# zju3dv/pats

Measured on AMD Instinct MI355X. Metric: image-pairs/sec (coarse+fine OT) on 640x480 MegaDepth; OT iters/sec per pair, higher is better.
Workload: dtype f32 (contractions: fp32 operands split into fp16 hi + lo, three exact-product MFMA passes, fp32 accumulate)

## Files before the change

### include/pats_amd.h

```cpp
#ifndef PATS_AMD_H
#define PATS_AMD_H

#include <stddef.h>
#include <stdint.h>

#ifdef __cplusplus
extern "C" {
#endif

typedef void* pats_stream_t;

enum {
    PATS_OK = 0,
    PATS_ERR_INVALID = 1,
    PATS_ERR_UNSUPPORTED = 2,
    PATS_ERR_LAUNCH = 3,
    PATS_ERR_NO_DEVICE = 4
};

enum { PATS_SINKHORN_AUTO = 0, PATS_SINKHORN_LOG = 1, PATS_SINKHORN_KERNEL = 2 };

const char* pats_version(void);
#define PATS_ABI_VERSION 8
int pats_abi_version(void);
const char* pats_last_error(void);
int pats_device_count(void);
int pats_set_sinkhorn_mode(int mode);
int pats_set_fine_fused(int on);

int pats_set_third_gather(int mode);

int pats_sinkhorn_fallbacks(int64_t* count, int reset);

int pats_sinkhorn_tail_solves(int64_t* count, int reset);

int pats_cost_f32(const float* d0, const float* d1, int64_t batch, int D, int n, int m, float* out,
                  pats_stream_t stream);

size_t pats_sinkhorn_workspace_bytes(int64_t batch, int M, int N);
int pats_sinkhorn_f32(const float* Z, int64_t batch, int M, int N, const float* log_mu,
                      const float* log_nu, int iters, float* out, void* workspace,
                      size_t workspace_bytes, pats_stream_t stream);

size_t pats_ot_workspace_bytes(int64_t batch, int M, int N);
int pats_log_optimal_transport_f32(const float* scores, int64_t batch, int m, int n,
                                   const float* alpha, const float* ns, int iters, float* Z,
                                   void* workspace, size_t workspace_bytes, pats_stream_t stream);

size_t pats_ot2_workspace_bytes(int64_t batch, int m, int n);
int pats_log_optimal_transport2_flags_f32(const float* scores, int64_t batch, int m, int n,
                                          const float* one, const float* ns, int iters, float bias_k,
                                          float* Z, uint8_t* col_nomatch, void* workspace,
                                          size_t workspace_bytes, pats_stream_t stream);
int pats_log_optimal_transport2_f32(const float* scores, int64_t batch, int m, int n,
                                    const float* one, const float* ns, int iters, float bias_k,
                                    float* Z, void* workspace, size_t workspace_bytes,
                                    pats_stream_t stream);

int pats_cost_ot_f32(const float* d0, const float* d1, int64_t batch, int D, int n, int m,
                     int variant, const float* scalar, const float* ns, int iters, float bias_k,
                     float* Z, void* workspace, size_t workspace_bytes, pats_stream_t stream);
size_t pats_cost_ot_workspace_bytes(int64_t batch, int D, int n, int m, int variant);
int pats_cost_ot_flags_f32(const float* d0, const float* d1, int64_t batch, int D, int n, int m,
                           int variant, const float* scalar, const float* ns, int iters, float bias_k,
                           float* Z, uint8_t* col_nomatch, void* workspace, size_t workspace_bytes,
                           pats_stream_t stream);

int pats_set_cost_ot_mid_event(void* event);

int pats_cost_ot_flags_counted_f32(const float* d0, const float* d1, int64_t batch_cap, const int64_t* batch_dev,
                                   int D, int n, int m, int variant, const float* scalar, const float* ns, int iters,
                                   float bias_k, float* Z, uint8_t* col_nomatch, void* workspace,
                                   size_t workspace_bytes, pats_stream_t stream);

int pats_colmass_sqrt_f32(const float* Z, int64_t batch, int M, int N, float* out,
                          pats_stream_t stream);
int pats_colmass_flags_f32(const float* Z, int64_t batch, int M, int N, float* out, uint8_t* col_nomatch,
                           pats_stream_t stream);
int pats_dustbin_bias_inplace_f32(float* Z, int64_t batch, int M, int N, float k,
                                  pats_stream_t stream);
int pats_exp_f32(const float* Z, int64_t count, float* out, pats_stream_t stream);

int pats_argmax_f32(const float* Z, int64_t batch, int M, int N, int64_t* row_arg,
                    int64_t* col_arg, pats_stream_t stream);

int pats_iterative_expand_f32(const float* P, int input_is_log, int64_t batch, int M, int N,
                              const float* scalex, const float* scaley, int lim3, int h, int w,
                              float lower_bound, int iter_num, float* whole_cost, float* core_cost,
                              float* average_point, float* x_scale, float* y_scale, int64_t* bound,
                              uint8_t* row_nomatch, pats_stream_t stream);

int pats_iterative_expand_counted_f32(const float* P, int input_is_log, int64_t batch_cap, const int64_t* batch_dev,
                                      int M, int N, const float* scalex, const float* scaley, int lim3, int h, int w,
                                      float lower_bound, int iter_num, float* whole_cost, float* core_cost,
                                      float* average_point, float* x_scale, float* y_scale, int64_t* bound,
                                      uint8_t* row_nomatch, pats_stream_t stream);

int pats_split_patches(const int32_t* sum_cycle_host, int height, int width, int max_once_used,
                       int64_t* second_layer_set, int64_t* third_layer_set);
int pats_split_patches_device(const int32_t* sum_cycle, int64_t pairs, int height, int width,
                              int max_once_used, int64_t* second_layer_set, int64_t* third_layer_set,
                              int32_t* cycle_num, pats_stream_t stream);

int pats_compute_imgs_bounds_f32(const float* x_scale, const float* y_scale,
                                 const float* average_point, const uint8_t* if_nomatching, int Np,
                                 int height, int width, int img, int64_t* bound5, int64_t* K_out,
                                 float* x_scale_new, float* y_scale_new, float* average_new,
                                 pats_stream_t stream);

int pats_left_crops_f32(const float* left, int n_img, int H, int W, const int64_t* bound5, int64_t K,
                        int height, int width, float* out, pats_stream_t stream);

int pats_compute_imgs_bounds_batch_f32(const float* x_scale, const float* y_scale, const float* average_point,
// ... 471 lines not shown
```

### pats_amd/_lib.py

```python
import ctypes
import os

_HERE = os.path.dirname(os.path.abspath(__file__))
LIB_PATH = os.path.join(_HERE, "libpats_amd.so")
if os.environ.get("PATS_AMD_DIAG_LIB", "") not in ("", "0"):
    _sfx = os.environ["PATS_AMD_DIAG_LIB"]
    LIB_PATH = os.path.join(_HERE, "libpats_amd_diag%s.so" % ("" if _sfx == "1" else _sfx))

c_void_p, c_int, c_i64, c_f, c_size = (ctypes.c_void_p, ctypes.c_int, ctypes.c_int64, ctypes.c_float,
                                       ctypes.c_size_t)

ABI_VERSION = 8



class PairTable(ctypes.Structure):
    _fields_ = [("pairs", ctypes.c_int64), ("shape_host", c_void_p), ("cell_base_host", c_void_p), ("shape", c_void_p),
                ("cell_base", c_void_p), ("img_base", c_void_p)]


_TAB = ctypes.POINTER(PairTable)


class CropFormat(ctypes.Structure):
    _fields_ = [("dtype", ctypes.c_int32), ("layout", ctypes.c_int32), ("normalize", ctypes.c_int32),
                ("mean", ctypes.c_float * 3), ("std", ctypes.c_float * 3)]


_FMT = ctypes.POINTER(CropFormat)

_SCORE_ARGS = [c_void_p, c_void_p, c_void_p, c_void_p, c_i64, c_void_p, c_i64, c_i64, c_void_p, c_i64, c_void_p, c_void_p, c_int, c_f,
               c_void_p, c_void_p, c_void_p, c_void_p, c_void_p, c_void_p, c_size, c_void_p]
_ADAPTIVE_ARGS = [ctypes.c_double, c_int, c_int, c_i64, c_void_p, c_void_p]
_POLISH_ARGS = [c_void_p, c_void_p, c_void_p, c_void_p, c_i64, c_void_p, c_i64, c_i64, c_void_p, c_void_p, c_int, c_f, c_void_p, c_i64,
                c_void_p, c_int, c_void_p, c_void_p, c_void_p, c_void_p, c_void_p, c_void_p, c_void_p, c_size, c_void_p]

SIGNATURES = {
    "pats_version": (ctypes.c_char_p, []),
    "pats_abi_version": (c_int, []),
    "pats_last_error": (ctypes.c_char_p, []),
    "pats_device_count": (c_int, []),
    "pats_set_sinkhorn_mode": (c_int, [c_int]),
    "pats_set_fine_fused": (c_int, [c_int]),
    "pats_set_third_gather": (c_int, [c_int]),
    "pats_sinkhorn_fallbacks": (c_int, [ctypes.POINTER(ctypes.c_int64), c_int]),
    "pats_sinkhorn_tail_solves": (c_int, [ctypes.POINTER(ctypes.c_int64), c_int]),
    "pats_set_gnn_redo_mode": (c_int, [c_int]),
    "pats_gnn_overflows": (c_int, [ctypes.POINTER(ctypes.c_int64), c_int]),
    "pats_cost_f32": (c_int, [c_void_p, c_void_p, c_i64, c_int, c_int, c_int, c_void_p, c_void_p]),
    "pats_sinkhorn_workspace_bytes": (c_size, [c_i64, c_int, c_int]),
    "pats_sinkhorn_f32": (c_int, [c_void_p, c_i64, c_int, c_int, c_void_p, c_void_p, c_int, c_void_p,
                                  c_void_p, c_size, c_void_p]),
    "pats_ot_workspace_bytes": (c_size, [c_i64, c_int, c_int]),
    "pats_log_optimal_transport_f32": (c_int, [c_void_p, c_i64, c_int, c_int, c_void_p, c_void_p, c_int,
                                               c_void_p, c_void_p, c_size, c_void_p]),
    "pats_ot2_workspace_bytes": (c_size, [c_i64, c_int, c_int]),
    "pats_log_optimal_transport2_f32": (c_int, [c_void_p, c_i64, c_int, c_int, c_void_p, c_void_p, c_int,
                                                c_f, c_void_p, c_void_p, c_size, c_void_p]),
    "pats_cost_ot_f32": (c_int, [c_void_p, c_void_p, c_i64, c_int, c_int, c_int, c_int, c_void_p,
                                 c_void_p, c_int, c_f, c_void_p, c_void_p, c_size, c_void_p]),
    "pats_cost_ot_flags_f32": (c_int, [c_void_p, c_void_p, c_i64, c_int, c_int, c_int, c_int, c_void_p,
                                       c_void_p, c_int, c_f, c_void_p, c_void_p, c_void_p, c_size, c_void_p]),
    "pats_set_cost_ot_mid_event": (c_int, [c_void_p]),
    "pats_cost_ot_flags_counted_f32": (c_int, [c_void_p, c_void_p, c_i64, c_void_p, c_int, c_int, c_int, c_int, c_void_p,
                                               c_void_p, c_int, c_f, c_void_p, c_void_p, c_void_p, c_size, c_void_p]),
    "pats_iterative_expand_counted_f32": (c_int, [c_void_p, c_int, c_i64, c_void_p, c_int, c_int, c_void_p, c_void_p, c_int,
                                                  c_int, c_int, c_f, c_int, c_void_p, c_void_p, c_void_p,
                                                  c_void_p, c_void_p, c_void_p, c_void_p, c_void_p]),
    "pats_fine_descriptors_counted_f32": (c_int, [c_void_p, c_void_p, c_void_p, c_void_p, c_void_p, c_i64, c_void_p, c_int,
                                                  c_void_p, c_void_p]),
    "pats_log_optimal_transport2_flags_f32": (c_int, [c_void_p, c_i64, c_int, c_int, c_void_p, c_void_p, c_int,
                                                      c_f, c_void_p, c_void_p, c_void_p, c_size, c_void_p]),
    "pats_colmass_flags_f32": (c_int, [c_void_p, c_i64, c_int, c_int, c_void_p, c_void_p, c_void_p]),
    "pats_cost_ot_workspace_bytes": (c_size, [c_i64, c_int, c_int, c_int, c_int]),
    "pats_colmass_sqrt_f32": (c_int, [c_void_p, c_i64, c_int, c_int, c_void_p, c_void_p]),
    "pats_dustbin_bias_inplace_f32": (c_int, [c_void_p, c_i64, c_int, c_int, c_f, c_void_p]),
    "pats_exp_f32": (c_int, [c_void_p, c_i64, c_void_p, c_void_p]),
    "pats_argmax_f32": (c_int, [c_void_p, c_i64, c_int, c_int, c_void_p, c_void_p, c_void_p]),
    "pats_iterative_expand_f32": (c_int, [c_void_p, c_int, c_i64, c_int, c_int, c_void_p, c_void_p, c_int,
                                          c_int, c_int, c_f, c_int, c_void_p, c_void_p, c_void_p,
                                          c_void_p, c_void_p, c_void_p, c_void_p, c_void_p]),
    "pats_split_patches": (c_int, [c_void_p, c_int, c_int, c_int, c_void_p, c_void_p]),
    "pats_split_patches_device": (c_int, [c_void_p, c_i64, c_int, c_int, c_int, c_void_p, c_void_p, c_void_p, c_void_p]),
    "pats_compute_imgs_bounds_batch_f32": (c_int, [c_void_p, c_void_p, c_void_p, c_void_p, c_int, c_int, c_int, c_int,
                                                   c_void_p, c_void_p, c_void_p, c_void_p, c_void_p, c_void_p, c_void_p]),
    "pats_left_crops_counted_f32": (c_int, [c_void_p, c_int, c_int, c_int, c_void_p, c_i64, c_void_p, c_int, c_int,
                                            c_void_p, c_void_p]),
    "pats_tensor_resize_hwc_counted_f32": (c_int, [c_void_p, c_int, c_int, c_int, c_int, c_void_p, c_i64, c_void_p,
                                                   c_void_p, c_void_p, c_void_p]),
    "pats_compute_imgs_bounds_f32": (c_int, [c_void_p, c_void_p, c_void_p, c_void_p, c_int, c_int, c_int,
                                             c_int, c_void_p, c_void_p, c_void_p, c_void_p, c_void_p,
                                             c_void_p]),
    "pats_left_crops_f32": (c_int, [c_void_p, c_int, c_int, c_int, c_void_p, c_i64, c_int, c_int, c_void_p,
                                    c_void_p]),
    "pats_tensor_resize_f32": (c_int, [c_void_p, c_int, c_int, c_int, c_int, c_void_p, c_i64, c_void_p,
                                       c_void_p, c_void_p]),
    "pats_tensor_resize_hwc_f32": (c_int, [c_void_p, c_int, c_int, c_int, c_int, c_void_p, c_i64,
                                           c_void_p, c_void_p, c_void_p]),
    "pats_compute_result_f32": (c_int, [c_void_p, c_int, c_i64, c_void_p, c_void_p, c_void_p, c_void_p,
                                        c_int, c_void_p, c_void_p, c_void_p, c_void_p, c_void_p,
                                        c_void_p]),
    "pats_compute_result_ws_f32": (c_int, [c_void_p, c_int, c_i64, c_void_p, c_void_p, c_void_p, c_void_p,
                                           c_int, c_void_p, c_void_p, c_void_p, c_void_p, c_void_p,
                                           c_void_p, c_size, c_void_p]),
    "pats_fine_descriptors_f32": (c_int, [c_void_p, c_void_p, c_void_p, c_void_p, c_void_p, c_i64, c_void_p, c_void_p]),
    "pats_third_descriptors_f32": (c_int, [c_void_p, c_void_p, c_void_p, c_void_p, c_void_p, c_void_p, c_void_p,
                                           c_i64, c_i64, c_void_p, c_void_p, c_void_p, c_void_p, c_void_p]),
    "pats_third_level_f32": (c_int, [c_void_p, c_void_p, c_i64, c_int, c_void_p, c_void_p, c_void_p, c_void_p,
                                     c_void_p, c_int, c_int, c_void_p, c_void_p, c_void_p, c_void_p, c_void_p,
                                     c_void_p]),
    "pats_third_descriptors_counted_f32": (c_int, [c_void_p, c_void_p, c_void_p, c_void_p, c_void_p, c_void_p, c_void_p,
                                                   c_i64, c_void_p, c_i64, c_void_p, c_void_p, c_void_p, c_void_p, c_void_p]),
    "pats_fine_descriptors_nhwc_f32": (c_int, [c_void_p, c_void_p, c_void_p, c_void_p, c_void_p, c_i64, c_void_p, c_void_p]),
    "pats_third_descriptors_nhwc_f32": (c_int, [c_void_p, c_void_p, c_void_p, c_void_p, c_void_p, c_void_p, c_void_p,
                                                c_i64, c_void_p, c_i64, c_void_p, c_void_p, c_void_p, c_void_p, c_void_p]),
    "pats_fine_descriptors_typed": (c_int, [c_void_p, c_void_p, c_void_p, c_int, c_int, c_void_p, c_void_p, c_i64, c_void_p,
                                            c_void_p, c_void_p]),
    "pats_third_descriptors_typed": (c_int, [c_void_p, c_void_p, c_int, c_int, c_void_p, c_void_p, c_void_p, c_void_p, c_void_p,
                                             c_i64, c_void_p, c_i64, c_void_p, c_void_p, c_void_p, c_void_p, c_void_p]),
    "pats_fine_descriptors_typed_out": (c_int, [c_void_p, c_void_p, c_void_p, c_int, c_int, c_void_p, c_void_p, c_i64, c_void_p,
                                                c_void_p, c_int, c_void_p]),
    "pats_third_descriptors_typed_out": (c_int, [c_void_p, c_void_p, c_int, c_int, c_void_p, c_void_p, c_void_p, c_void_p,
                                                 c_void_p, c_i64, c_void_p, c_i64, c_void_p, c_void_p, c_int, c_void_p, c_void_p,
                                                 c_void_p]),
    "pats_third_level_counted_f32": (c_int, [c_void_p, c_void_p, c_i64, c_void_p, c_int, c_void_p, c_void_p, c_void_p,
                                             c_void_p, c_void_p, c_int, c_int, c_void_p, c_void_p, c_void_p, c_void_p,
                                             c_void_p]),
# ... 107 lines not shown
    "pats_epipolar_pose_by_pair_f64": (c_int, [c_void_p, c_void_p, c_void_p, c_void_p, c_i64, c_void_p, c_i64, c_i64, c_void_p, c_void_p,
                                               c_void_p, c_i64, c_void_p, c_void_p, c_int, c_void_p, c_void_p, c_void_p, c_void_p,
                                               c_void_p, c_void_p, c_void_p, c_void_p, c_void_p, c_size, c_void_p]),
    "pats_epipolar_triangulate_workspace_bytes": (c_size, [c_i64, c_i64]),
    "pats_epipolar_triangulate_by_pair_f64": (c_int, [c_void_p, c_void_p, c_void_p, c_i64, c_void_p, c_i64, c_i64, c_void_p, c_void_p,
                                                      c_void_p, c_void_p, c_int, c_void_p, c_void_p, c_void_p, c_void_p, c_void_p,
                                                      c_void_p, c_void_p, c_void_p, c_void_p, c_void_p, c_size, c_void_p]),
    "pats_pose_error_by_pair_f64": (c_int, [c_void_p, c_void_p, c_void_p, c_void_p, c_void_p, c_i64, c_i64, ctypes.c_double, c_void_p,
                                            c_void_p, c_void_p, c_void_p, c_void_p]),
    "pats_pose_auc_max_n": (c_i64, []),
    "pats_pose_auc_f64": (c_int, [c_void_p, c_i64, c_void_p, c_i64, c_void_p, c_void_p, c_void_p, c_void_p]),
    "pats_homography_hypotheses_workspace_bytes": (c_size, [c_i64, c_i64]),
    "pats_homography_hypotheses_by_pair_f32": (c_int, [c_void_p, c_void_p, c_void_p, c_i64, c_void_p, c_i64, c_i64, c_i64, c_void_p,
                                                       c_void_p, c_int, c_void_p, c_void_p, c_void_p, c_size, c_void_p]),
    "pats_homography_score_workspace_bytes": (c_size, [c_i64, c_i64, c_i64]),
    "pats_homography_score_by_pair_f32": (c_int, [c_void_p, c_void_p, c_void_p, c_void_p, c_i64, c_void_p, c_i64, c_i64, c_void_p, c_i64,
                                                  c_void_p, c_void_p, c_int, c_f, c_void_p, c_void_p, c_void_p, c_void_p, c_void_p,
                                                  c_void_p, c_size, c_void_p]),
    "pats_homography_refit_workspace_bytes": (c_size, [c_i64]),
    "pats_homography_refit_by_pair_f64": (c_int, [c_void_p, c_void_p, c_void_p, c_i64, c_void_p, c_void_p, c_i64, c_int, c_void_p,
                                                  c_void_p, c_void_p, c_void_p, c_size, c_void_p]),
    "pats_homography_pose_workspace_bytes": (c_size, [c_i64, c_i64]),
    "pats_homography_pose_by_pair_f64": (c_int, [c_void_p, c_void_p, c_void_p, c_void_p, c_i64, c_void_p, c_i64, c_i64, c_void_p, c_void_p,
                                                 c_void_p, c_i64, c_void_p, c_void_p, c_void_p, c_int, ctypes.c_double] + [c_void_p] * 14 +
                                         [c_void_p, c_size, c_void_p]),
    "pats_pose_select_workspace_bytes": (c_size, [c_i64, c_i64]),
    "pats_pose_select_by_pair": (c_int, [c_void_p, c_i64, c_void_p, c_i64, c_i64] + [c_void_p] * 23 + [c_void_p, c_size, c_void_p]),
    "pats_epipolar_score_adaptive_workspace_bytes": (c_size, [c_i64, c_i64, c_i64]),
    "pats_epipolar_score_adaptive_by_pair_f32": (c_int, _SCORE_ARGS + _ADAPTIVE_ARGS),
    "pats_homography_score_adaptive_workspace_bytes": (c_size, [c_i64, c_i64, c_i64]),
    "pats_homography_score_adaptive_by_pair_f32": (c_int, _SCORE_ARGS + _ADAPTIVE_ARGS),
    "pats_msac_gain_one": (c_i64, []),
    "pats_epipolar_score_msac_by_pair_f32": (c_int, _SCORE_ARGS + [c_void_p, c_void_p]),
    "pats_homography_score_msac_by_pair_f32": (c_int, _SCORE_ARGS + [c_void_p, c_void_p]),
    "pats_epipolar_polish_workspace_bytes": (c_size, [c_i64, c_i64, c_i64]),
    "pats_epipolar_polish_by_pair_f32": (c_int, _POLISH_ARGS),
    "pats_homography_polish_workspace_bytes": (c_size, [c_i64, c_i64, c_i64]),
    "pats_homography_polish_by_pair_f32": (c_int, _POLISH_ARGS),
    "pats_epipolar_hypotheses7_workspace_bytes": (c_size, [c_i64, c_i64]),
    "pats_epipolar_hypotheses7_by_pair_f32": (c_int, [c_void_p, c_void_p, c_void_p, c_i64, c_void_p, c_i64, c_i64, c_i64, c_void_p,
                                                      c_void_p, c_int, c_void_p, c_void_p, c_void_p, c_void_p, c_size, c_void_p]),
    "pats_fundamental_refit_workspace_bytes": (c_size, [c_i64]),
    "pats_fundamental_refit_by_pair_f64": (c_int, [c_void_p, c_void_p, c_void_p, c_i64, c_void_p, c_void_p, c_i64, c_int, c_void_p,
                                                   c_void_p, c_void_p, c_void_p, c_void_p, c_void_p, c_size, c_void_p]),
    "pats_fundamental_polish_workspace_bytes": (c_size, [c_i64, c_i64, c_i64]),
    "pats_fundamental_polish_by_pair_f32": (c_int, _POLISH_ARGS),
    "pats_conv1x1_workspace_bytes": (c_size, []),
    "pats_conv1x1_f32": (c_int, [c_void_p, c_void_p, c_void_p, c_i64, c_int, c_int, c_int, c_void_p, c_void_p, c_void_p,
                                 c_void_p, c_void_p, c_size, c_void_p]),
    "pats_bn_fold_workspace_bytes": (c_size, [c_int]),
    "pats_bn_fold_f32": (c_int, [c_void_p, c_i64, c_int, c_int, c_void_p, c_void_p, c_f, c_void_p, c_void_p, c_void_p,
                                 c_size, c_void_p]),
    "pats_scale_head_f32": (c_int, [c_void_p, c_i64, c_int, c_int, c_int, c_int, c_void_p, c_void_p, c_int, c_void_p, c_void_p,
                                    c_void_p]),
    "pats_get_result_workspace_bytes": (c_size, [c_i64, c_i64, c_i64]),
    "pats_get_result_f32": (c_int, [c_int, c_void_p, c_void_p, c_i64, c_void_p, c_void_p, c_void_p, c_void_p, c_i64,
                                    ctypes.POINTER(c_int), ctypes.POINTER(c_int), c_void_p, c_void_p, c_void_p,
                                    c_void_p, c_i64, c_void_p, c_void_p, c_size, c_void_p]),
}

_lib = None


def lib():
    global _lib
    if _lib is None:
        if not os.path.exists(LIB_PATH):
            raise ImportError(
                "pats_amd: %s is missing - the HIP extension was not built (run "
                "`python -m pats_amd.build` / __graft_entry__.build()). There is no CPU fallback."
                % LIB_PATH)
        try:
            import torch
        except ImportError:
            pass
        handle = ctypes.CDLL(LIB_PATH)
        for name, (res, args) in SIGNATURES.items():
            fn = getattr(handle, name)
            fn.restype = res
            fn.argtypes = args
        if handle.pats_abi_version() != ABI_VERSION:
            raise ImportError("pats_amd: %s exports ABI %d, these bindings were written for ABI %d - rebuild the library "
                              "(python -m pats_amd.build)" % (LIB_PATH, handle.pats_abi_version(), ABI_VERSION))
        _lib = handle
    return _lib


def check(rc, what):
    if rc != 0:
        msg = lib().pats_last_error().decode()
        raise RuntimeError("pats_amd.%s failed (code %d): %s" % (what, rc, msg))
```

### pats_amd/csrc/expand.hip

```cpp
#include "common.hpp"
#include "third_device.hpp"

namespace pats {

struct ExpandArgs {
    const float* P;
    int input_is_log;
    int64_t rows_total;
    int M, N;
    const float* scalex;
    const float* scaley;
    int lim3, h, w;
    float lower_bound;
    int iter_num;
    float *whole_cost, *core_cost, *average_point, *x_scale, *y_scale;
    int64_t* bound;
    uint8_t* row_nomatch;
    const int64_t* live;
};

__device__ __forceinline__ float range_val(int d, int k) { return k <= d ? (float)k : 1e7f; }

__device__ __forceinline__ int clamp_seq(float f, int wh, int S) {
    return (f >= 0.f && f <= (float)(wh - 1)) ? (int)f : S;
}


template <bool SMALL>
__global__ void __launch_bounds__(256)
expand_kernel(ExpandArgs a) {
    extern __shared__ __attribute__((aligned(16))) float sm[];
    const int t = threadIdx.x & 15, slot = threadIdx.x >> 4;
    const int ROWS_PER_WG = blockDim.x >> 4;
    const int M = a.M, N = a.N, m = M - 1, n = N - 1;
    int64_t rows_total = a.rows_total;
    if (a.live) {
        const int64_t lv = *a.live * m;
        rows_total = lv < rows_total ? lv : rows_total;
        if ((int64_t)blockIdx.x * ROWS_PER_WG >= rows_total) return;
    }
    const int64_t gr_raw = (int64_t)blockIdx.x * ROWS_PER_WG + slot;
    const bool active = gr_raw < rows_total;
    const int64_t gr = active ? gr_raw : rows_total - 1;
    const int64_t b = gr / m;
    const int r = (int)(gr - b * m);
    const int ld = N + 3;
    float* prow = sm + (size_t)slot * ld;
    float* popp = sm + (size_t)ROWS_PER_WG * ld + (size_t)slot * ld;
    const float* Pb = a.P + b * (int64_t)M * N;
    const float* src = Pb + (int64_t)r * N;
    const float* oppsrc = Pb + (int64_t)(M - 1) * N;
    const float* sx = a.scalex + b * (int64_t)n;
    const float* sy = a.scaley + b * (int64_t)n;
    float fv = -INFINITY;
    int fi = 0x7fffffff;
    const int64_t g0 = (int64_t)blockIdx.x * ROWS_PER_WG;
    const int64_t glast = min(g0 + ROWS_PER_WG - 1, rows_total - 1);
    const int64_t b0 = g0 / m;
    const bool shared_opp = glast / m - b0 <= 1;
    if (shared_opp) {
        popp = sm + (size_t)ROWS_PER_WG * ld + (size_t)(b - b0) * ld;
        for (int e = threadIdx.x; e < 2 * N; e += blockDim.x) {
            const int which = e >= N, j = e - which * N;
            const int64_t bb = min(b0 + which, (int64_t)(rows_total - 1) / m);
            const float o = a.P[bb * (int64_t)M * N + (int64_t)(M - 1) * N + j];
            sm[(size_t)ROWS_PER_WG * ld + (size_t)which * ld + j] = a.input_is_log ? expf(o) : o;
        }
    }
    float bv = -INFINITY, bva = -INFINITY;
    int bi = 0x7fffffff, bia = 0x7fffffff;
    float rowsum = 0.f;
    for (int j = t; j < N; j += 16) {
        const float x0 = src[j];
        if (x0 > fv || fi == 0x7fffffff) { fv = x0; fi = j; }
        const float x = a.input_is_log ? expf(x0) : x0;
        prow[j] = x;
        rowsum += x;
        if (j < N - 1 && (x > bv || bi == 0x7fffffff)) { bv = x; bi = j; }
        if (x > bva || bia == 0x7fffffff) { bva = x; bia = j; }
        if (!shared_opp) {
            const float o = oppsrc[j];
            popp[j] = a.input_is_log ? expf(o) : o;
        }
    }
    if (a.row_nomatch) {
        row16_argmax(fv, fi);
        if (t == 0 && active) a.row_nomatch[gr] = fi == N - 1;
    }
    if (t == 0) { prow[N] = ZERO_F; popp[N] = ZERO_F; }
    wg_barrier();

    const int width = a.h > a.w ? a.h : a.w;
    const int height = (a.h * a.w) / width;
    const int wh = width * height, S = wh + 1;
    auto ES = [&](int idx) { return prow[idx]; };
    auto ESC = [&](int idx) { return idx < n ? sx[idx] * sy[idx] : ZERO_F; };
    auto EOPP = [&](int idx) { return popp[idx]; };

    row16_argmax(bv, bi);
    row16_argmax(bva, bia);
    const float the_scale = row16_sum(rowsum);
    const int max0 = bi;
    const bool if_nomatching = (bia == m);
    float last_nomatching = EOPP(max0);
    int up = max0 / a.lim3, down = up, left = max0 % a.lim3, right = left;
    int bd0 = 0, bd1 = 0, sb0 = 0, sb1 = 0;
    float last_sum = ES(max0);

    for (int it = 0; it < a.iter_num; ++it) {
        sb0 = bd0; sb1 = bd1;
        const float off[4] = {(float)(left + up * width - width),
                              (float)(left + down * width + width),
                              (float)(left + up * width - 1),
                              (float)(right + up * width + 1)};
        float es[4], nm[4], sc[4];
        float vcell[4];
        int scell[4];
#pragma unroll
        for (int d = 0; d < 4; ++d) {
            float e = 0.f, q = 0.f, c = 0.f;
            auto cell = [&](int k) {
                const float f = d < 2 ? range_val(sb1, k) + off[d] : range_val(sb0, k) * (float)width + off[d];
                const int s = clamp_seq(f, wh, S);
                const float v = ES(s);
                e += v;
                if (SMALL) { vcell[d] = v; scell[d] = s; }
                else {
                    q += (v > a.lower_bound) ? EOPP(s) : ZERO_F;
                    c += ESC(s);
                }
            };
            if (SMALL) { vcell[d] = 0.f; scell[d] = S; if (t < width) cell(t); }
            else for (int k = t; k < width; k += 16) cell(k);
            es[d] = row16_sum(e);
            if (!SMALL) { nm[d] = row16_sum(q); sc[d] = row16_sum(c); }
        }
        if (up == 0) es[0] = ZERO_F;
        if (down == height - 1) es[1] = ZERO_F;
        if (left == 0) es[2] = ZERO_F;
        if (right == width - 1) es[3] = ZERO_F;
        int arg = 0;
        float mx = es[0];
#pragma unroll
        for (int d = 1; d < 4; ++d)
            if (es[d] > mx) { mx = es[d]; arg = d; }
        float mnm;
        if (SMALL) {
            float v = vcell[0];
            int sidx = scell[0];
#pragma unroll
            for (int d = 1; d < 4; ++d)
                if (arg == d) { v = vcell[d]; sidx = scell[d]; }
            const float q = (t < width) ? ((v > a.lower_bound) ? EOPP(sidx) : ZERO_F) : 0.f;
            mnm = row16_sum(q);
        } else {
            mnm = nm[0];
#pragma unroll
            for (int d = 1; d < 4; ++d)
                if (arg == d) mnm = nm[d];
        }
        (void)sc;
        float add_sum = ZERO_F, add_nm = ZERO_F;
        if (mx > a.lower_bound) {
            up -= (arg == 0);
            down += (arg == 1);
            left -= (arg == 2);
            right += (arg == 3);
            add_sum = mx;
            add_nm = mnm;
        }
        bd0 = down - up;
        bd1 = right - left;
        last_sum = last_sum + add_sum;
        last_nomatching = last_nomatching + add_nm;
    }
    const bool if_core_exist = (bd0 > 1) && (bd1 > 1);

    float e4, s4;
    {
        const float eoff[4] = {(float)(left + up * width), (float)(left + down * width),
                               (float)(left + up * width), (float)(right + up * width)};
        float ed[4], sd[4];
#pragma unroll
        for (int d = 0; d < 4; ++d) {
            float e = 0.f, c = 0.f;
            auto cell = [&](int k) {
                const float f = d < 2 ? range_val(sb1, k) + eoff[d]
                                      : range_val(sb0, k) * (float)width + eoff[d];
                const int s = clamp_seq(f, wh, S);
                e += ES(s);
                c += ESC(s);
            };
            if (SMALL) { if (t < width) cell(t); }
            else for (int k = t; k < width; k += 16) cell(k);
            ed[d] = row16_sum(e);
            sd[d] = row16_sum(c);
        }
        e4 = (ed[0] + ed[1]) + (ed[2] + ed[3]);
        s4 = (sd[0] + sd[1]) + (sd[2] + sd[3]);
    }

    float wx = 0.f, wy = 0.f, sumx = 0.f, sumy = 0.f, ws = 0.f, so = 0.f;
    const int q16 = 16 / a.w, r16 = 16 - q16 * a.w;
    int pyi = t / a.w, pxi = t - pyi * a.w;
    const bool no_cell = up > (n - 1) / a.w || left > a.w - 1;
    for (int p = t; p < n; p += 16, pyi += q16, pxi += r16) {
        if (pxi >= a.w) { pxi -= a.w; ++pyi; }
        const bool crit = pyi >= up && pyi <= down && pxi >= left && pxi <= right;
        if (!__any(crit || no_cell)) continue;
        const float fx = sx[p], fy = sy[p];
        float ox = ZERO_F, oy = ZERO_F;
        if (crit) {
            const float root = sqrtf(prow[p] + 1e-7f);
            ox = root / fx;
            oy = root / fy;
        }
        wx += ox * (float)pxi;
        wy += oy * (float)pyi;
        sumx += ox;
        sumy += oy;
        const float o = ox * oy;
        ws += o * (fx * fy);
        so += o;
    }
    wx = row16_sum(wx); wy = row16_sum(wy); sumx = row16_sum(sumx); sumy = row16_sum(sumy);
    ws = row16_sum(ws); so = row16_sum(so);

    if (t == 0 && active) {
        const int corner[4] = {up * width + left, up * width + right, down * width + left,
                               down * width + right};
        float cps = 0.f, css = 0.f;
#pragma unroll
        for (int q = 0; q < 4; ++q) {
            int s = corner[q];
            if (!(s >= 0)) s = S;
            if (!(s <= wh - 1)) s = S;
            cps += ES(s);
            css += ESC(s);
        }
        const float core_scale_sum = the_scale - s4 + css;
        const float core_sum = last_sum - e4 + cps;
        a.core_cost[gr] = (if_core_exist && !if_nomatching)
                              ? fabsf((core_sum - core_scale_sum) / the_scale) : ZERO_F;
        a.whole_cost[gr] = if_nomatching ? ZERO_F
            : (fabsf(the_scale - last_sum) + last_nomatching / 4.0f) / the_scale;
        a.average_point[gr * 2 + 1] = wx / sumx + 0.5f;
        a.average_point[gr * 2 + 0] = wy / sumy + 0.5f;
        const float average_scale = sqrtf(ws / so);
        a.x_scale[gr] = 1.0f / (average_scale / 1.0f);
        a.y_scale[gr] = 1.0f / (average_scale * 1.0f);
        a.bound[gr * 4 + 0] = up;
        a.bound[gr * 4 + 1] = down;
        a.bound[gr * 4 + 2] = left;
        a.bound[gr * 4 + 3] = right;
    }
}

}

using namespace pats;

static int expand_impl(const float* P, int input_is_log, int64_t batch, int M, int N, const float* scalex, const float* scaley,
                       int lim3, int h, int w, float lower_bound, int iter_num, float* whole_cost, float* core_cost,
                       float* average_point, float* x_scale, float* y_scale, int64_t* bound, uint8_t* row_nomatch,
                       const int64_t* live, pats_stream_t stream);

extern "C" int pats_iterative_expand_f32(const float* P, int input_is_log, int64_t batch, int M,
                                         int N, const float* scalex, const float* scaley, int lim3,
                                         int h, int w, float lower_bound, int iter_num,
                                         float* whole_cost, float* core_cost, float* average_point,
                                         float* x_scale, float* y_scale, int64_t* bound,
                                         uint8_t* row_nomatch, pats_stream_t stream) {
    return expand_impl(P, input_is_log, batch, M, N, scalex, scaley, lim3, h, w, lower_bound, iter_num, whole_cost, core_cost,
                       average_point, x_scale, y_scale, bound, row_nomatch, nullptr, stream);
}

extern "C" int pats_iterative_expand_counted_f32(const float* P, int input_is_log, int64_t batch_cap, const int64_t* batch_dev,
                                                 int M, int N, const float* scalex, const float* scaley, int lim3, int h, int w,
                                                 float lower_bound, int iter_num, float* whole_cost, float* core_cost,
                                                 float* average_point, float* x_scale, float* y_scale, int64_t* bound,
                                                 uint8_t* row_nomatch, pats_stream_t stream) {
    PATS_REQUIRE(batch_dev, "iterative_expand_counted: null count");
    return expand_impl(P, input_is_log, batch_cap, M, N, scalex, scaley, lim3, h, w, lower_bound, iter_num, whole_cost, core_cost,
                       average_point, x_scale, y_scale, bound, row_nomatch, batch_dev, stream);
}

static int expand_impl(const float* P, int input_is_log, int64_t batch, int M, int N, const float* scalex, const float* scaley,
                       int lim3, int h, int w, float lower_bound, int iter_num, float* whole_cost, float* core_cost,
                       float* average_point, float* x_scale, float* y_scale, int64_t* bound, uint8_t* row_nomatch,
                       const int64_t* live, pats_stream_t stream) {
    PATS_REQUIRE(batch >= 0 && M > 1 && N > 1 && h > 0 && w > 0 && lim3 > 0 && iter_num >= 1,
                 "iterative_expand: bad argument");
    PATS_REQUIRE(h * w == N - 1, "iterative_expand: grid %dx%d does not match %d target columns", h,
                 w, N - 1);
    if (batch == 0) return PATS_OK;
    PATS_REQUIRE(P && scalex && scaley && whole_cost && core_cost && average_point && x_scale &&
                     y_scale && bound, "iterative_expand: null pointer");
    ExpandArgs a{P, input_is_log, batch * (int64_t)(M - 1), M, N, scalex, scaley, lim3, h, w,
                 lower_bound, iter_num, whole_cost, core_cost, average_point, x_scale, y_scale, bound, row_nomatch, live};
    int rows_per_wg = 16;
    size_t lds = 2 * (size_t)rows_per_wg * (size_t)(N + 3) * sizeof(float);
    if (lds > 48 * 1024) {
        rows_per_wg = 4;
        lds = 2 * (size_t)rows_per_wg * (size_t)(N + 3) * sizeof(float);
    }
    PATS_REQUIRE(lds <= 64 * 1024, "iterative_expand: N=%d too large", N);
    const int64_t blocks = ceil_div(a.rows_total, rows_per_wg);
    if (h <= 16 && w <= 16)
        hipLaunchKernelGGL(expand_kernel<true>, dim3((unsigned)blocks), dim3(16 * rows_per_wg), lds, as_stream(stream), a);
    else
        hipLaunchKernelGGL(expand_kernel<false>, dim3((unsigned)blocks), dim3(16 * rows_per_wg), lds, as_stream(stream), a);
    return check_launch("expand_kernel");
}
```

### pats_amd/ops.py

```python
import ctypes

import numpy as np
import torch

from . import _lib

_L = _lib.lib
_check = _lib.check
_L()


_raw_stream = getattr(torch._C, "_cuda_getCurrentRawStream", None)


def _stream():
    if _raw_stream is not None:
        return ctypes.c_void_p(_raw_stream(torch.cuda.current_device()))
    return ctypes.c_void_p(torch.cuda.current_stream().cuda_stream)


def _dev(t, name, dtype=torch.float32):
    if not isinstance(t, torch.Tensor):
        raise TypeError("%s must be a torch.Tensor" % name)
    if not t.is_cuda:
# ... 27 lines not shown
            raise RuntimeError("pats_amd: %s must be float32, float16 or bfloat16, got %s" % (name, t.dtype))
    dtypes = {t.dtype for t in tensors}
    if dtypes == {torch.float32}:
        return [_map(t, n) for t, n in zip(tensors, names)], _MAP_DTYPES[torch.float32]
    if len(dtypes) != 1:
        return [_map(t.float(), n) for t, n in zip(tensors, names)], _MAP_DTYPES[torch.float32]
    dt = tensors[0].dtype
    maps = [_map(t, n, dt) for t, n in zip(tensors, names)]
    if len({cl for _, cl in maps}) != 1:
        maps = [(t.contiguous(), False) for t, _ in maps]
    align = 16 if maps[0][1] else 4
    if any(t.data_ptr() % align for t, _ in maps):
        return [_map(t.float(), n) for t, n in zip(tensors, names)], _MAP_DTYPES[torch.float32]
    return maps, _MAP_DTYPES[dt]


def _descs_any(tensors, names):
    for t, name in zip(tensors, names):
        if not isinstance(t, torch.Tensor):
            raise TypeError("%s must be a torch.Tensor" % name)
        if t.dtype not in _MAP_DTYPES:
            raise RuntimeError("pats_amd: %s must be float32, float16 or bfloat16, got %s" % (name, t.dtype))
    dtypes = {t.dtype for t in tensors}
    if len(dtypes) == 1 and torch.float32 not in dtypes:
        dt = tensors[0].dtype
        descs = [_dev(t, n, dt) for t, n in zip(tensors, names)]
        if not any(t.data_ptr() % t.element_size() for t in descs):
            return descs, _MAP_DTYPES[dt]
    return [_dev(t.float(), n) for t, n in zip(tensors, names)], _MAP_DTYPES[torch.float32]


def _ptr(t):
    return ctypes.c_void_p(t.data_ptr()) if t is not None else ctypes.c_void_p(0)


_WS = {}
_WS_MAX = 64 << 20
_WS_ON = [False]


class workspace_cache:

    def __enter__(self):
        self.prev = _WS_ON[0]
        _WS_ON[0] = True

    def __exit__(self, *exc):
        _WS_ON[0] = self.prev


def _workspace(nbytes, device):
    n = max(int(nbytes), 1)
    if not _WS_ON[0] or n > _WS_MAX or _raw_stream is None or torch.cuda.is_current_stream_capturing():
        return torch.empty(n, dtype=torch.uint8, device=device)
    key = (device.index, _raw_stream(torch.cuda.current_device()))
    t = _WS.get(key)
    if t is None or t.numel() < n:
        t = _WS[key] = torch.empty(min(_WS_MAX, max(2 * n, 1 << 20)), dtype=torch.uint8, device=device)
    return t


def _scalar_dev(x, device):
    if isinstance(x, torch.Tensor):
        return x.detach().reshape(1).to(device=device, dtype=torch.float32)
    return torch.full((1,), float(x), dtype=torch.float32, device=device)


def set_sinkhorn_mode(mode):
    names = {"auto": 0, "log": 1, "kernel": 2}
    prev = _L().pats_set_sinkhorn_mode(names[mode])
    return {v: k for k, v in names.items()}[prev]


def set_fine_fused(on):
    return bool(_L().pats_set_fine_fused(1 if on else 0))


def set_third_gather(mode):
    modes = {"tile": 0, "point": 1}
    if mode not in modes:
        raise ValueError("set_third_gather: mode must be 'tile' or 'point'")
    prev = _L().pats_set_third_gather(modes[mode])
    return {v: k for k, v in modes.items()}.get(prev, "tile")


def sinkhorn_fallbacks(reset=True):
    import ctypes
    n = ctypes.c_int64(0)
    rc = _L().pats_sinkhorn_fallbacks(ctypes.byref(n), 1 if reset else 0)
    if rc != 0:
        raise RuntimeError(_L().pats_last_error().decode())
    return int(n.value)


def sinkhorn_tail_solves(reset=True):
    n = ctypes.c_int64(0)
    _check(_L().pats_sinkhorn_tail_solves(ctypes.byref(n), 1 if reset else 0), "sinkhorn_tail_solves")
    return int(n.value)


def set_gnn_redo(mode):
    names = {"inline": 0, "deferred": 1}
    prev = _L().pats_set_gnn_redo_mode(names[mode])
    return {v: k for k, v in names.items()}[prev]


def gnn_overflows(reset=True):
    n = ctypes.c_int64(0)
    _check(_L().pats_gnn_overflows(ctypes.byref(n), 1 if reset else 0), "gnn_overflows")
    return bool(n.value)


def cost(mdesc0, mdesc1, out=None):
    (d0, d1), code = _descs_any([mdesc0, mdesc1], ["mdesc0", "mdesc1"])
    b, D, n = d0.shape
    if d1.shape[0] != b or d1.shape[1] != D:
        raise RuntimeError("cost: descriptor shapes %s / %s do not match" % (tuple(d0.shape), tuple(d1.shape)))
    m = d1.shape[2]
    if out is None:
        out = torch.empty((b, n, m), dtype=torch.float32, device=d0.device)
    elif tuple(out.shape) != (b, n, m) or out.dtype != torch.float32 or not out.is_contiguous() or out.device != d0.device:
        raise RuntimeError("cost: out must be a contiguous float32 [%d, %d, %d] tensor on %s" % (b, n, m, d0.device))
    if code:
        _check(_L().pats_cost_typed(_ptr(d0), _ptr(d1), code, b, D, n, m, _ptr(out), _stream()), "cost")
    else:
        _check(_L().pats_cost_f32(_ptr(d0), _ptr(d1), b, D, n, m, _ptr(out), _stream()), "cost")
    return out


def log_sinkhorn_iterations(Z, log_mu, log_nu, iters: int):
    Z, log_mu, log_nu = _dev(Z, "Z"), _dev(log_mu, "log_mu"), _dev(log_nu, "log_nu")
    b, M, N = Z.shape
    if tuple(log_mu.shape) != (b, M) or tuple(log_nu.shape) != (b, N):
        raise RuntimeError("log_sinkhorn_iterations: marginal shapes do not match Z")
    out = torch.empty_like(Z)
    nb = _L().pats_sinkhorn_workspace_bytes(b, M, N)
    ws = _workspace(nb, Z.device)
    _check(_L().pats_sinkhorn_f32(_ptr(Z), b, M, N, _ptr(log_mu), _ptr(log_nu), int(iters), _ptr(out),
                                  _ptr(ws), nb, _stream()), "log_sinkhorn_iterations")
    return out


def log_optimal_transport(scores, alpha, ns, iters: int):
    scores = _dev(scores, "scores")
    b, m, n = scores.shape
    ns = _dev(ns, "ns")
    if ns.numel() != b * n:
        raise RuntimeError("log_optimal_transport: ns must have %d entries per batch" % n)
    ns = ns.reshape(b, n)
    a = _scalar_dev(alpha, scores.device)
    Z = torch.empty((b, m + 1, n + 1), dtype=torch.float32, device=scores.device)
    nb = _L().pats_ot_workspace_bytes(b, m + 1, n + 1)
    ws = _workspace(nb, scores.device)
    _check(_L().pats_log_optimal_transport_f32(_ptr(scores), b, m, n, _ptr(a), _ptr(ns), int(iters),
                                               _ptr(Z), _ptr(ws), nb, _stream()), "log_optimal_transport")
    return Z


def log_optimal_transport2(scores, one, ns, iters: int, bias_k: float = 0.0):
    scores = _dev(scores, "scores")
    b, m, n = scores.shape
    ns = _dev(ns, "ns")
    if ns.numel() != b * (n - 1):
        raise RuntimeError("log_optimal_transport2: ns must have %d entries per batch" % (n - 1))
    ns = ns.reshape(b, n - 1)
    o = _scalar_dev(one, scores.device)
# ... 2117 lines not shown
```

Before: 1909.

## Compact still-growing patches in expand kernel to cut divergent iterative growth

```diff
diff --git a/include/pats_amd.h b/include/pats_amd.h
--- a/include/pats_amd.h
+++ b/include/pats_amd.h
@@ -29,6 +29,8 @@
 int pats_set_fine_fused(int on);
 
 int pats_set_third_gather(int mode);
+
+int pats_set_expand_compact(int on);
 
 int pats_sinkhorn_fallbacks(int64_t* count, int reset);
 
diff --git a/pats_amd/_lib.py b/pats_amd/_lib.py
--- a/pats_amd/_lib.py
+++ b/pats_amd/_lib.py
@@ -43,6 +43,7 @@
     "pats_set_sinkhorn_mode": (c_int, [c_int]),
     "pats_set_fine_fused": (c_int, [c_int]),
     "pats_set_third_gather": (c_int, [c_int]),
+    "pats_set_expand_compact": (c_int, [c_int]),
     "pats_sinkhorn_fallbacks": (c_int, [ctypes.POINTER(ctypes.c_int64), c_int]),
     "pats_sinkhorn_tail_solves": (c_int, [ctypes.POINTER(ctypes.c_int64), c_int]),
     "pats_set_gnn_redo_mode": (c_int, [c_int]),
@@ -316,6 +317,8 @@
         if handle.pats_abi_version() != ABI_VERSION:
             raise ImportError("pats_amd: %s exports ABI %d, these bindings were written for ABI %d - rebuild the library "
                               "(python -m pats_amd.build)" % (LIB_PATH, handle.pats_abi_version(), ABI_VERSION))
+        if os.environ.get("PATS_EXPAND_COMPACT", "") == "0":
+            handle.pats_set_expand_compact(0)
         _lib = handle
     return _lib
 
diff --git a/pats_amd/csrc/expand.hip b/pats_amd/csrc/expand.hip
--- a/pats_amd/csrc/expand.hip
+++ b/pats_amd/csrc/expand.hip
@@ -1,5 +1,6 @@
 #include "common.hpp"
 #include "third_device.hpp"
+#include <type_traits>
 
 namespace pats {
 
@@ -26,9 +27,26 @@
 }
 
 
-template <bool SMALL>
-__global__ void __launch_bounds__(256)
+constexpr int STAGE_LOADS = 10;
+
+struct Grow {
+    int up, down, left, right;
+    int bd0, bd1, sb0, sb1;
+    float last_sum, last_nomatching;
+};
+
+constexpr int ST_WORDS = 11;
+enum { ST_UP, ST_DOWN, ST_LEFT, ST_RIGHT, ST_SB0, ST_SB1, ST_SUM, ST_NM, ST_SCALE, ST_NOMATCH, ST_OPP };
+
+constexpr size_t expand_lds_floats(int rows_per_wg, int N, int compact) {
+    return compact ? (size_t)(compact + 2) * (size_t)(N + 3) + (size_t)compact * ST_WORDS + (size_t)compact + (size_t)(compact / 4) * compact + 4 * (size_t)(N - 1)
+                   : 2 * (size_t)rows_per_wg * (size_t)(N + 3);
+}
+
+template <bool SMALL, int COMPACT>
+__global__ void __launch_bounds__(COMPACT ? 16 * COMPACT : 256)
 expand_kernel(ExpandArgs a) {
+    static_assert(COMPACT == 0 || (SMALL && COMPACT % 4 == 0 && COMPACT <= 64), "one ballot covers a workgroup's patches");
     extern __shared__ __attribute__((aligned(16))) float sm[];
     const int t = threadIdx.x & 15, slot = threadIdx.x >> 4;
     const int ROWS_PER_WG = blockDim.x >> 4;
@@ -40,8 +58,8 @@
         if ((int64_t)blockIdx.x * ROWS_PER_WG >= rows_total) return;
     }
     const int64_t gr_raw = (int64_t)blockIdx.x * ROWS_PER_WG + slot;
-    const bool active = gr_raw < rows_total;
-    const int64_t gr = active ? gr_raw : rows_total - 1;
+    bool active = gr_raw < rows_total;
+    int64_t gr = active ? gr_raw : rows_total - 1;
     const int64_t b = gr / m;
     const int r = (int)(gr - b * m);
     const int ld = N + 3;
@@ -57,8 +75,25 @@
     const int64_t g0 = (int64_t)blockIdx.x * ROWS_PER_WG;
     const int64_t glast = min(g0 + ROWS_PER_WG - 1, rows_total - 1);
     const int64_t b0 = g0 / m;
-    const bool shared_opp = glast / m - b0 <= 1;
-    if (shared_opp) {
+    const bool shared_opp = COMPACT || glast / m - b0 <= 1;
+    constexpr int WG_THREADS = COMPACT ? 16 * COMPACT : 256;
+    constexpr int OPP_LOADS = (2 * 257 + WG_THREADS - 1) / WG_THREADS, SCALE_LOADS = (4 * 256 + WG_THREADS - 1) / WG_THREADS;
+    float* scales = sm + (size_t)(COMPACT + 2) * ld + (size_t)COMPACT * ST_WORDS + COMPACT + (COMPACT / 4) * COMPACT;
+    float oin[OPP_LOADS], sin_[SCALE_LOADS];
+    if constexpr (COMPACT != 0) {
+        popp = sm + (size_t)COMPACT * ld + (size_t)(b - b0) * ld;
+        const int64_t blast = (rows_total - 1) / m;
+#pragma unroll
+        for (int c = 0; c < OPP_LOADS; ++c) {
+            const int e = min((int)threadIdx.x + c * WG_THREADS, 2 * N - 1), which = e >= N, j = e - which * N;
+            oin[c] = a.P[min(b0 + which, blast) * (int64_t)M * N + (int64_t)(M - 1) * N + j];
+        }
+#pragma unroll
+        for (int c = 0; c < SCALE_LOADS; ++c) {
+            const int e = min((int)threadIdx.x + c * WG_THREADS, 4 * n - 1), which = e >= 2 * n, rest = e - which * 2 * n, xy = rest >= n;
+            sin_[c] = (xy ? a.scaley : a.scalex)[min(b0 + which, blast) * (int64_t)n + rest - xy * n];
+        }
+    } else if (shared_opp) {
         popp = sm + (size_t)ROWS_PER_WG * ld + (size_t)(b - b0) * ld;
         for (int e = threadIdx.x; e < 2 * N; e += blockDim.x) {
             const int which = e >= N, j = e - which * N;
@@ -70,18 +105,43 @@
     float bv = -INFINITY, bva = -INFINITY;
     int bi = 0x7fffffff, bia = 0x7fffffff;
     float rowsum = 0.f;
-    for (int j = t; j < N; j += 16) {
-        const float x0 = src[j];
-        if (x0 > fv || fi == 0x7fffffff) { fv = x0; fi = j; }
-        const float x = a.input_is_log ? expf(x0) : x0;
-        prow[j] = x;
-        rowsum += x;
-        if (j < N - 1 && (x > bv || bi == 0x7fffffff)) { bv = x; bi = j; }
-        if (x > bva || bia == 0x7fffffff) { bva = x; bia = j; }
-        if (!shared_opp) {
-            const float o = oppsrc[j];
-            popp[j] = a.input_is_log ? expf(o) : o;
-        }
+    auto stage = [&](int jb, auto loads) {
+        constexpr int LOADS = decltype(loads)::value;
+        float xin[LOADS];
+#pragma unroll
+        for (int c = 0; c < LOADS; ++c) xin[c] = src[min(jb + 16 * c, N - 1)];
+#pragma unroll
+        for (int c = 0; c < LOADS; ++c) {
+            const int j = jb + 16 * c;
+            if (j >= N) break;
+            const float x0 = xin[c];
+            if (x0 > fv || fi == 0x7fffffff) { fv = x0; fi = j; }
+            const float x = a.input_is_log ? expf(x0) : x0;
+            prow[j] = x;
+            rowsum += x;
+            if (j < N - 1 && (x > bv || bi == 0x7fffffff)) { bv = x; bi = j; }
+            if (x > bva || bia == 0x7fffffff) { bva = x; bia = j; }
+            if (!shared_opp) {
+                const float o = oppsrc[j];
+                popp[j] = a.input_is_log ? expf(o) : o;
+            }
+        }
+    };
+    if constexpr (SMALL) {
+        stage(t, std::integral_constant<int, STAGE_LOADS>());
+        if (N > 16 * STAGE_LOADS) stage(t + 16 * STAGE_LOADS, std::integral_constant<int, 17 - STAGE_LOADS>());
+    } else {
+        for (int jb = t; jb < N; jb += 16 * STAGE_LOADS) stage(jb, std::integral_constant<int, STAGE_LOADS>());
+    }
+    if constexpr (COMPACT != 0) {
+#pragma unroll
+        for (int c = 0; c < OPP_LOADS; ++c) {
+            const int e = threadIdx.x + c * WG_THREADS, which = e >= N, j = e - which * N;
+            if (e < 2 * N) sm[(size_t)(COMPACT + which) * ld + j] = a.input_is_log ? expf(oin[c]) : oin[c];
+        }
+#pragma unroll
+        for (int c = 0; c < SCALE_LOADS; ++c)
+            if ((int)threadIdx.x + c * WG_THREADS < 4 * n) scales[threadIdx.x + c * WG_THREADS] = sin_[c];
     }
     if (a.row_nomatch) {
         row16_argmax(fv, fi);
@@ -99,20 +159,22 @@
 
     row16_argmax(bv, bi);
     row16_argmax(bva, bia);
-    const float the_scale = row16_sum(rowsum);
+    float the_scale = row16_sum(rowsum);
     const int max0 = bi;
-    const bool if_nomatching = (bia == m);
-    float last_nomatching = EOPP(max0);
-    int up = max0 / a.lim3, down = up, left = max0 % a.lim3, right = left;
-    int bd0 = 0, bd1 = 0, sb0 = 0, sb1 = 0;
-    float last_sum = ES(max0);
-
-    for (int it = 0; it < a.iter_num; ++it) {
-        sb0 = bd0; sb1 = bd1;
-        const float off[4] = {(float)(left + up * width - width),
-                              (float)(left + down * width + width),
-                              (float)(left + up * width - 1),
-                              (float)(right + up * width + 1)};
+    bool if_nomatching = (bia == m);
+    Grow g;
+    g.last_nomatching = EOPP(max0);
+    g.up = g.down = max0 / a.lim3;
+    g.left = g.right = max0 % a.lim3;
+    g.bd0 = g.bd1 = g.sb0 = g.sb1 = 0;
+    g.last_sum = ES(max0);
+
+    auto grow_step = [&](const float* row, const float* opp, Grow& g) -> bool {
+        g.sb0 = g.bd0; g.sb1 = g.bd1;
+        const float off[4] = {(float)(g.left + g.up * width - width),
+                              (float)(g.left + g.down * width + width),
+                              (float)(g.left + g.up * width - 1),
+                              (float)(g.right + g.up * width + 1)};
         float es[4], nm[4], sc[4];
         float vcell[4];
         int scell[4];
@@ -120,13 +182,13 @@
         for (int d = 0; d < 4; ++d) {
             float e = 0.f, q = 0.f, c = 0.f;
             auto cell = [&](int k) {
-                const float f = d < 2 ? range_val(sb1, k) + off[d] : range_val(sb0, k) * (float)width + off[d];
+                const float f = d < 2 ? range_val(g.sb1, k) + off[d] : range_val(g.sb0, k) * (float)width + off[d];
                 const int s = clamp_seq(f, wh, S);
-                const float v = ES(s);
+                const float v = row[s];
                 e += v;
                 if (SMALL) { vcell[d] = v; scell[d] = s; }
                 else {
-                    q += (v > a.lower_bound) ? EOPP(s) : ZERO_F;
+                    q += (v > a.lower_bound) ? opp[s] : ZERO_F;
                     c += ESC(s);
                 }
             };
@@ -135,10 +197,10 @@
             es[d] = row16_sum(e);
             if (!SMALL) { nm[d] = row16_sum(q); sc[d] = row16_sum(c); }
         }
-        if (up == 0) es[0] = ZERO_F;
-        if (down == height - 1) es[1] = ZERO_F;
-        if (left == 0) es[2] = ZERO_F;
-        if (right == width - 1) es[3] = ZERO_F;
+        if (g.up == 0) es[0] = ZERO_F;
+        if (g.down == height - 1) es[1] = ZERO_F;
+        if (g.left == 0) es[2] = ZERO_F;
+        if (g.right == width - 1) es[3] = ZERO_F;
         int arg = 0;
         float mx = es[0];
 #pragma unroll
@@ -151,7 +213,7 @@
 #pragma unroll
             for (int d = 1; d < 4; ++d)
                 if (arg == d) { v = vcell[d]; sidx = scell[d]; }
-            const float q = (t < width) ? ((v > a.lower_bound) ? EOPP(sidx) : ZERO_F) : 0.f;
+            const float q = (t < width) ? ((v > a.lower_bound) ? opp[sidx] : ZERO_F) : 0.f;
             mnm = row16_sum(q);
         } else {
             mnm = nm[0];
@@ -161,19 +223,68 @@
         }
         (void)sc;
         float add_sum = ZERO_F, add_nm = ZERO_F;
-        if (mx > a.lower_bound) {
-            up -= (arg == 0);
-            down += (arg == 1);
-            left -= (arg == 2);
-            right += (arg == 3);
+        const bool grew = mx > a.lower_bound;
+        if (grew) {
+            g.up -= (arg == 0);
+            g.down += (arg == 1);
+            g.left -= (arg == 2);
+            g.right += (arg == 3);
             add_sum = mx;
             add_nm = mnm;
         }
-        bd0 = down - up;
-        bd1 = right - left;
-        last_sum = last_sum + add_sum;
-        last_nomatching = last_nomatching + add_nm;
-    }
+        g.bd0 = g.down - g.up;
+        g.bd1 = g.right - g.left;
+        g.last_sum = g.last_sum + add_sum;
+        g.last_nomatching = g.last_nomatching + add_nm;
+        return grew;
+    };
+
+    if constexpr (COMPACT == 0) {
+        for (int it = 0; it < a.iter_num; ++it) grow_step(prow, popp, g);
+    } else {
+        int* st = reinterpret_cast<int*>(sm + (size_t)(COMPACT + 2) * ld);
+        int* grew0 = st + COMPACT * ST_WORDS;
+        int* order = grew0 + COMPACT + (threadIdx.x >> 6) * COMPACT;
+        const bool grew = grow_step(prow, popp, g);
+        if (t == 0) {
+            int* s = st + slot * ST_WORDS;
+            s[ST_UP] = g.up; s[ST_DOWN] = g.down; s[ST_LEFT] = g.left; s[ST_RIGHT] = g.right;
+            s[ST_SB0] = g.sb0; s[ST_SB1] = g.sb1;
+            s[ST_SUM] = __float_as_int(g.last_sum); s[ST_NM] = __float_as_int(g.last_nomatching);
+            s[ST_SCALE] = __float_as_int(the_scale); s[ST_NOMATCH] = if_nomatching; s[ST_OPP] = (int)(b - b0);
+            grew0[slot] = grew && active && a.iter_num > 1;
+        }
+        wg_barrier();
+        const int lane = threadIdx.x & 63;
+        const bool on = lane < COMPACT && grew0[lane] != 0;
+        const unsigned long long growing = __builtin_amdgcn_ballot_w64(on), below = (1ull << lane) - 1ull;
+        const int count = __popcll(growing);
+        if (lane < COMPACT) order[on ? __popcll(growing & below) : count + __popcll(~growing & below)] = lane;
+        wave_lds_sync();
+        const int p = order[slot];
+        const int* s = st + p * ST_WORDS;
+        g.up = s[ST_UP]; g.down = s[ST_DOWN]; g.left = s[ST_LEFT]; g.right = s[ST_RIGHT];
+        g.sb0 = s[ST_SB0]; g.sb1 = s[ST_SB1];
+        g.bd0 = g.down - g.up; g.bd1 = g.right - g.left;
+        g.last_sum = __int_as_float(s[ST_SUM]); g.last_nomatching = __int_as_float(s[ST_NM]);
+        the_scale = __int_as_float(s[ST_SCALE]);
+        if_nomatching = s[ST_NOMATCH] != 0;
+        active = g0 + p < rows_total;
+        gr = active ? g0 + p : rows_total - 1;
+        prow = sm + (size_t)p * ld;
+        popp = sm + (size_t)(COMPACT + s[ST_OPP]) * ld;
+        sx = scales + (size_t)s[ST_OPP] * 2 * n;
+        sy = sx + n;
+        int k = 1;
+        if (slot < count)
+            for (bool more = true; k < a.iter_num && more; ++k) more = grow_step(prow, popp, g);
+        for (; k < a.iter_num; ++k) {
+            g.last_sum = g.last_sum + ZERO_F;
+            g.last_nomatching = g.last_nomatching + ZERO_F;
+        }
+    }
+    const int up = g.up, down = g.down, left = g.left, right = g.right, bd0 = g.bd0, bd1 = g.bd1, sb0 = g.sb0, sb1 = g.sb1;
+    const float last_sum = g.last_sum, last_nomatching = g.last_nomatching;
     const bool if_core_exist = (bd0 > 1) && (bd1 > 1);
 
     float e4, s4;
@@ -260,6 +371,14 @@
 
 using namespace pats;
 
+static int g_expand_compact = 1;
+extern "C" int pats_set_expand_compact(int on) {
+    const int prev = g_expand_compact;
+    if (on == 0 || on == 1) g_expand_compact = on;
+    return prev;
+}
+constexpr int EXPAND_COMPACT_ROWS = 16;
+
 static int expand_impl(const float* P, int input_is_log, int64_t batch, int M, int N, const float* scalex, const float* scaley,
                        int lim3, int h, int w, float lower_bound, int iter_num, float* whole_cost, float* core_cost,
                        float* average_point, float* x_scale, float* y_scale, int64_t* bound, uint8_t* row_nomatch,
@@ -298,6 +417,14 @@
                      y_scale && bound, "iterative_expand: null pointer");
     ExpandArgs a{P, input_is_log, batch * (int64_t)(M - 1), M, N, scalex, scaley, lim3, h, w,
                  lower_bound, iter_num, whole_cost, core_cost, average_point, x_scale, y_scale, bound, row_nomatch, live};
+    const bool small = h <= 16 && w <= 16;
+    const size_t lds_compact = expand_lds_floats(0, N, EXPAND_COMPACT_ROWS) * sizeof(float);
+    if (small && iter_num > 1 && M >= EXPAND_COMPACT_ROWS && lds_compact <= 48 * 1024 && g_expand_compact) {
+        const int64_t blocks = ceil_div(a.rows_total, EXPAND_COMPACT_ROWS);
+        hipLaunchKernelGGL((expand_kernel<true, EXPAND_COMPACT_ROWS>), dim3((unsigned)blocks), dim3(16 * EXPAND_COMPACT_ROWS), lds_compact,
+                           as_stream(stream), a);
+        return check_launch("expand_kernel");
+    }
     int rows_per_wg = 16;
     size_t lds = 2 * (size_t)rows_per_wg * (size_t)(N + 3) * sizeof(float);
     if (lds > 48 * 1024) {
@@ -306,9 +433,9 @@
     }
     PATS_REQUIRE(lds <= 64 * 1024, "iterative_expand: N=%d too large", N);
     const int64_t blocks = ceil_div(a.rows_total, rows_per_wg);
-    if (h <= 16 && w <= 16)
-        hipLaunchKernelGGL(expand_kernel<true>, dim3((unsigned)blocks), dim3(16 * rows_per_wg), lds, as_stream(stream), a);
+    if (small)
+        hipLaunchKernelGGL((expand_kernel<true, 0>), dim3((unsigned)blocks), dim3(16 * rows_per_wg), lds, as_stream(stream), a);
     else
-        hipLaunchKernelGGL(expand_kernel<false>, dim3((unsigned)blocks), dim3(16 * rows_per_wg), lds, as_stream(stream), a);
+        hipLaunchKernelGGL((expand_kernel<false, 0>), dim3((unsigned)blocks), dim3(16 * rows_per_wg), lds, as_stream(stream), a);
     return check_launch("expand_kernel");
 }
diff --git a/pats_amd/ops.py b/pats_amd/ops.py
--- a/pats_amd/ops.py
+++ b/pats_amd/ops.py
@@ -133,6 +133,10 @@
         raise ValueError("set_third_gather: mode must be 'tile' or 'point'")
     prev = _L().pats_set_third_gather(modes[mode])
     return {v: k for k, v in modes.items()}.get(prev, "tile")
+
+
+def set_expand_compact(on):
+    return bool(_L().pats_set_expand_compact(1 if on else 0))
 
 
 def sinkhorn_fallbacks(reset=True):
```

Measured after the change: 1952, median of 6. About the same (+2.2%).
